# crabml/crabml

Hardware: AMD Instinct MI355X
Metric: decode tokens/sec (batch-1 greedy), Llama-3-8B shape Q4_0 (higher is better)
Workload: dtype q4_0 x q8_0 -> i32 dot, f32 accumulate

## Files before the change

crabml_amd/csrc/fused.hip:

```cpp
#include <algorithm>
#include <chrono>
#include <thread>
#include <cmath>

#include "fused_common.hpp"
#include "fused_attention.hpp"
#include "fused_ffn.hpp"
#include "sampler.hpp"
#include "prefill_rows.hpp"
#include "lazy.hpp"


#include <dlfcn.h>

using namespace crabml_hip;

struct crabml_hip_tp_comm {
  crabml_hip_device* dev = nullptr;
  void* nccl = nullptr;
  int nranks = 1, rank = 0;
  bool p2p = false;
  bool connected = false;
  unsigned long long* inbox = nullptr;
  bool via_ipc[8] = {false};
// ... 214 lines not shown
  return t;
}

hipError_t raise_dyn_lds(const crabml_hip_device* dev, const void* fn, int bytes) {
  static std::mutex mu;
  static std::map<std::pair<int, const void*>, int> have;
  if (dev->dry) return hipErrorNoDevice;
  std::lock_guard<std::mutex> g(mu);
  int& cur = have[{dev->ordinal, fn}];
  if (bytes <= cur) return hipSuccess;
  const hipError_t e = hipFuncSetAttribute(fn, hipFuncAttributeMaxDynamicSharedMemorySize, bytes);
  if (e == hipSuccess) cur = bytes;
  return e;
}

int dalloc(crabml_hip_llama* c, size_t bytes, void** out) {
  size_t cap = 0;
  CH_TRY(pool_alloc(c->dev, bytes, out, &cap));
  c->allocs.push_back({*out, cap});
  return 0;
}

Planes planes_of(const crabml_hip_buf* b) {
  return Planes{(const i32x4*)b->ptr, scale_plane<unsigned short>(b)};
}

struct ActPtrs {
  signed char* q;
  unsigned short* d;
  void* isum;
};
ActPtrs act_ptrs(char* p, size_t n, uint32_t qt) {
  ActLayout al = act_layout(qt, n);
  return ActPtrs{(signed char*)p, (unsigned short*)(p + al.off_d), (void*)(p + al.off_aux)};
}
template <int FMT>
typename ActOf<FMT>::type act_view(const ActPtrs& a) {
  ActLayout al;
  al.off_d = (size_t)((const char*)a.d - (const char*)a.q);
  al.off_aux = (size_t)((const char*)a.isum - (const char*)a.q);
  return act_at<typename ActOf<FMT>::type>((const char*)a.q, al);
}

int n_segments(const crabml_hip_llama* c) { return 2 * (int)c->cfg.n_layers + 1; }

int chunk_split(uint64_t flags, int k, int dim, int n_cu, bool x_only = false) {
  return (flags & CRABML_HIP_LLAMA_SPLIT_CHUNKS_ALWAYS)  ? 2
         : (flags & CRABML_HIP_LLAMA_SPLIT_CHUNKS_NEVER) ? 1
         : (k / 32 >= 256 && dim / 32 <= n_cu)           ? 2
         : (x_only && dim / 32 <= n_cu)                  ? 2
                                                         : 1;
}

int norm_nit(int dim) { return dim <= 4096 ? 4 : 12; }
void launch_norm_f32(hipStream_t st, float* x, const float* addv, const float* wn, int dim, float eps, float* out, int half) {
  with_const_else<4, 12>(norm_nit(dim), [&](auto nit) {
    k_norm_f32<decltype(nit)::value><<<1, 1024, norm_lds_bytes(dim), st>>>(x, addv, wn, dim, eps, out, half);
  });
}

typedef decltype(&k_attn_pv_split<1>) PvSplitFn;
struct PvSplitKernel {
  PvSplitFn fn = nullptr;
  int nsub = 0, threads = 0;
  size_t lds = 0;
};
PvSplitKernel pv_split_kernel(int grp) {
  PvSplitKernel k;
  with_const<1, 2, 4, 6, 8>(grp, [&](auto g) {
    typedef PvSplit<decltype(g)::value> P;
    k = PvSplitKernel{k_attn_pv_split<decltype(g)::value>, P::NSUB, P::THREADS, P::LDS};
  });
  return k;
}
typedef decltype(&k_attn_s<0>) AttnSFn;
AttnSFn attn_s_kernel(int hd) { return hd == 128 ? k_attn_s<128> : k_attn_s<0>; }
typedef decltype(&k_attn_flash_rows<64>) FlashRowsFn;
FlashRowsFn flash_rows_kernel(int hd) { return hd == 128 ? k_attn_flash_rows<128> : hd == 64 ? k_attn_flash_rows<64> : nullptr; }
typedef decltype(&k_gemv_res_nq<CRABML_HIP_Q4_K, 1, 1, false, false, true>) NqOrdKFn;
NqOrdKFn nq_ord_k_kernel(int split, int qin) {
  NqOrdKFn fn = nullptr;
  with_const_else<2, 1>(split, [&](auto s) {
    with_const_else<2, 1>(qin, [&](auto q) { fn = k_gemv_res_nq<CRABML_HIP_Q4_K, decltype(s)::value, decltype(q)::value, false, false, true>; });
  });
  return fn;
}
typedef FmtList<CRABML_HIP_Q4_K, CRABML_HIP_Q5_K, CRABML_HIP_Q6_K, CRABML_HIP_Q3_K, CRABML_HIP_Q2_K> KBodies;
struct KBodyRow {
  int fmt;
  bool epi_only;
  bool v_whole;
  int n_alt;
  int alt[2];
  bool takes(uint32_t t) const {
    for (int i = 0; i < n_alt; i++)
      if ((uint32_t)alt[i] == t) return true;
    return false;
  }
};
template <int FMT, int... ALT>
constexpr KBodyRow k_body_row(FmtList<ALT...>) {
  return KBodyRow{FMT, KBody<FMT>::EPI_ONLY, KBody<FMT>::V_WHOLE, (int)sizeof...(ALT), {ALT...}};
}
template <int... FMTS>
const KBodyRow* k_body_of(FmtList<FMTS...>, uint32_t t) {
  static constexpr KBodyRow rows[] = {k_body_row<FMTS>(typename KBody<FMTS>::VAlt{})...};
// ... 240 lines not shown
      k_sample_pick<true><<<1, SAMPLE_PICK_THREADS, 0, st>>>(c->sm_keys, n, c->sm_hist, ss);
    else
      k_sample_pick<false><<<1, SAMPLE_PICK_THREADS, 0, st>>>(c->sm_keys, n, c->sm_hist, ss);
    CH_HIP(dev, hipGetLastError());
    return 0;
  }
  k_argmax_partial<<<ARGMAX_BLOCKS, 256, 0, st>>>(out, c->vocab_l, c->am_val, c->am_idx, c->vocab_off);
  if (c->split_vocab && c->comm && c->comm->p2p)
    k_argmax_step_tp<<<1, 64, 0, st>>>(c->am_val, c->am_idx, ARGMAX_BLOCKS, token_d, pos_d, step_d, c->out_tokens, c->out_cap, c->state + 4,
                                       tp_view(c, true), n_segments(c));
  else
    k_argmax_step<<<1, 64, 0, st>>>(c->am_val, c->am_idx, ARGMAX_BLOCKS, token_d, pos_d, step_d, c->out_tokens, c->out_cap, c->state + 4,
                                    c->split_vocab ? c->am_best : (int*)nullptr);
  CH_HIP(dev, hipGetLastError());
  return 0;
}

static QkvEpiB qwen2_epi(const crabml_hip_llama* c, const QkvEpi& e, int l) {
  return QkvEpiB{e, (const float*)c->bq[l]->ptr, (const float*)c->bk[l]->ptr, (const float*)c->bv[l]->ptr};
}
template <class E>
struct QkvArchOf {
  static constexpr int value = QKV_LLAMA;
};
template <>
struct QkvArchOf<QkvEpiB> {
  static constexpr int value = QKV_QWEN2;
};
template <>
struct QkvArchOf<QkvEpiN> {
  static constexpr int value = QKV_GEMMA;
};
template <class F>
void with_qkv_epi(const crabml_hip_llama* c, const QkvEpi& e, int l, F&& f) {
  if (c->qwen2)
    f(qwen2_epi(c, e, l));
  else if (c->gemma)
    f(QkvEpiN{e});
  else
    f(e);
}
QkvEpi decode_qkv_epi(const crabml_hip_llama* c, int l) {
  return QkvEpi{c->qbuf, c->kc[l], c->vc[l], c->rope, c->state + 1, 1.0f / std::sqrt((float)c->hd), c->dim_l, c->kv_dim_l, c->hd,
                (int)c->cfg.rope_dim, c->npairs, (int)c->cfg.seq_len, c->cfg.use_f16_kv_cache ? 1 : 0};
}
void launch_embed(const crabml_hip_llama* c) {
  const int dim = (int)c->cfg.embedding_dim;
  k_embed<<<(dim + 255) / 256, 256, 0, c->dev->stream>>>((const char*)c->token_embed->ptr, (int)c->token_embed->dtype,
                                                         c->token_embed->wl.off_scale, c->state, dim, c->x, c->embed_scale);
}

template <int QIN, bool TP = false, bool DEFER = false>
struct NqForm {};
template <int FMT, int SPLIT, int QIN, bool TP, bool DEFER>
constexpr auto nq_kernel(NqForm<QIN, TP, DEFER>) {
  return &k_gemv_res_nq<FMT, SPLIT, QIN, TP, DEFER>;
}

template <int FMT>
int enqueue_segment_t(crabml_hip_llama* c, int seg) {
  crabml_hip_device* dev = c->dev;
  hipStream_t st = dev->stream;
  const auto& g = c->cfg;
  const int dim = (int)g.embedding_dim, hd = c->hd;
  const int dim_l = c->dim_l, kv_dim_l = c->kv_dim_l, hidden_l = c->hidden_l;
  const int n_heads_l = c->n_heads_l;
  const bool tp = c->tp > 1;
  const int L = (int)g.n_layers;
  constexpr bool Q81 = FMT == CRABML_HIP_Q4_1;
  const uint32_t qt = c->qt;
  ActPtrs ad = act_ptrs(c->act_dim, dim, qt), aa = act_ptrs(c->act_attn, dim_l, qt), ah = act_ptrs(c->act_hid, hidden_l, qt);
  const bool prof = dev->prof_on && !c->use_graph && !c->capturing;
  const double blk_b = (double)block_bytes(c->wtype) / 32.0;
  auto P0 = [&](crabml_hip_device::ProfRec* r, uint32_t stage, double rows, double k) {
    return prof ? prof_begin(dev, r, c->wtype, stage, rows * k * blk_b + 4.0 * k + 4.0 * rows) : 0;
  };
  auto P1 = [&](crabml_hip_device::ProfRec* r) { return prof ? prof_end(dev, r) : 0; };
  crabml_hip_device::ProfRec pr{};
  crabml_hip_device::ProfRec* R = prof ? &pr : nullptr;
  const bool do_pf = !(g.flags & CRABML_HIP_LLAMA_NO_PREFETCH);
  auto plan = [&](const crabml_hip_buf* a, const crabml_hip_buf* b, const crabml_hip_buf* cc) {
    PrefetchPlan pf{};
    const crabml_hip_buf* v[3] = {a, b, cc};
    for (int i = 0; i < 3; i++) {
      pf.p[i] = do_pf && v[i] ? v[i]->ptr : nullptr;
      pf.n[i] = do_pf && v[i] ? (v[i]->wl.total / 16) * 16 : 0;
    }
    pf.sink = c->state + 3;
    return pf;
  };
  const int spare = do_pf ? (dev->n_cu > 1 ? dev->n_cu - 1 : 0) : 0;
  const size_t norm_lds = norm_lds_bytes(dim);
  auto norm_quant = [&](const float* wn, float eps, bool add_pending, const PrefetchPlan& pf) {
    crabml_hip_device::ProfRec nr{};
    if (prof) prof_begin(dev, &nr, CRABML_HIP_F32, 6, 8.0 * dim);
    const float* addv = add_pending ? c->partial : nullptr;
    with_const_else<4, 12>(norm_nit(dim), [&](auto nit) {
      launch_k(st, prof ? &nr : nullptr, k_norm_quant<decltype(nit)::value, Q81>, dim3(1 + spare), dim3(1024), norm_lds, c->x, addv, wn, dim, eps, ad.q,
               ad.d, ad.isum, pf, c->plan.ordered ? 0 : 1);
    });
    if (prof) prof_end(dev, &nr);
  };
  const bool norm_epi = c->plan.norm_epi;
  static const int qkv_upfront = test_hook_off("CRABML_HIP_QKV_UPFRONT") ? 0 : 1;
  const bool defer_wo = c->plan.defer_norm && !Q81;
  const bool defer_down = c->plan.defer_norm && !Q81;
  auto gemv_out = [&](const crabml_hip_buf* w, const ActPtrs& a, int k, uint32_t stage, const float* wnext, float eps_next, bool defer = false,
                      const float* xin = nullptr) -> int {
    CH_TRY(P0(&pr, stage, dim, k));
    float* dst = tp ? c->partial : c->x;
    if (norm_epi) {
      NormGather ng{c->slots, c->slots + dim / 16, c->state + 4, c->state + 5, n_segments(c), seg, c->rsums};
      const int split = chunk_split(g.flags, k, dim, dev->n_cu);
      c->tap.note(seg / 2, stage == 2 ? CRABML_HIP_PLAN_SPLIT_WO : CRABML_HIP_PLAN_SPLIT_DOWN, split);
      const TpP2P tpv = tp_view(c, tp);
      auto nq = [&](auto form, size_t lds, const float* rhs, auto tparg) {
        with_const_else<2, 1>(split, [&](auto s) {
          launch_k(st, R, nq_kernel<FMT, decltype(s)::value>(form), dim3(dim / 32 * split), dim3(1024), lds, planes_of(w), act_view<FMT>(a), rhs, c->x,
                   wnext, eps_next, ad.q, ad.d, ad.isum, ng, k / 32, Planes6{nullptr, 0}, tparg);
        });
      };
      if (xin != nullptr && !Q81) {
        if constexpr (!Q81) {
          if (tpv.n > 1)
            nq(NqForm<1, true>{}, q8_0_lds_bytes(k / 32), xin, tpv);
          else
            nq(NqForm<1>{}, q8_0_lds_bytes(k / 32), xin, NoTp{});
        }
      } else if (tpv.n > 1) {
        nq(NqForm<0, true>{}, 0, nullptr, tpv);
      } else if (c->plan.ordered) {
        static const int pipe_mode = test_hook_int("CRABML_HIP_ORD_PIPE", -1);
        const int pipe = pipe_mode >= 0 ? pipe_mode : FMT == CRABML_HIP_Q8_0 ? 2 : 1;
        const bool piped = pipe >= (split == 2 ? 1 : 2);
        with_const_else<2, 1>(split, [&](auto s) {
          with_const_else<0, 1>(piped, [&](auto p) {
            launch_k(st, R, k_gemv_res_nq_ord<FMT, decltype(s)::value, decltype(p)::value != 0>, dim3(dim / 32 * split), dim3(1024),
                     nq_ord_lds_bytes(k / 32, split), planes_of(w), act_view<FMT>(a), c->x, wnext, eps_next, ad.q, ad.d, ad.isum, ng, k / 32);
          });
        });
      } else if (defer && !Q81) {
        if constexpr (!Q81) nq(NqForm<0, false, true>{}, 0, nullptr, NoTp{});
      } else {
        nq(NqForm<0>{}, 0, nullptr, NoTp{});
      }
    } else if (c->plan.ordered) {
      launch_k(st, R, k_gemv_res_ord<FMT>, dim3((dim + 7) / 8), dim3(256), ord_terms_lds_bytes(k / 32), planes_of(w), act_view<FMT>(a), c->x, dim, k / 32);
    } else if (tp) {
      launch_k(st, R, k_gemv_res<FMT, 1, false>, dim3((dim + 1) / 2), dim3(128), 0, planes_of(w), act_view<FMT>(a), dst, dim, k / 32);
    } else {
      launch_k(st, R, k_gemv_res<FMT, 1, true>, dim3((dim + 1) / 2), dim3(128), 0, planes_of(w), act_view<FMT>(a), dst, dim, k / 32);
    }
    CH_TRY(P1(&pr));
    return 0;
  };

  const size_t ad_bytes = act_layout(qt, (size_t)dim).total, rs_bytes = c->rsums ? (size_t)(dim / 32) * 4 : 0;
  TapRec& tap = c->tap;
  auto TAP = [&](bool on, int f, const void* src, size_t bytes) -> int { return on ? tap.copy(c, f, src, bytes) : 0; };
  if (seg == 2 * L) {
    const void* cls_act = c->act_dim;
    if (c->out_qt != qt) {
      const float* addv = tp && !norm_epi ? c->partial : nullptr;
      launch_norm_f32(st, c->x, addv, (const float*)c->rms_final->ptr, dim, g.rms_norm_eps, c->xn, c->plan.ordered ? 0 : 1);
      if (c->out_qt == CRABML_HIP_F32) {
        cls_act = c->xn;
      } else {
        launch_quantize_act(st, c->out_qt, c->xn, (size_t)dim, c->act_dim);
      }
    } else if (!norm_epi) {
      norm_quant((const float*)c->rms_final->ptr, g.rms_norm_eps, tp, plan(nullptr, nullptr, nullptr));
      CH_TRY(TAP(tap.layer == L - 1, CRABML_HIP_TAP_DOWN_ACT, c->act_dim, ad_bytes));
// ... 2278 lines not shown
```

crabml_amd/csrc/fused_ffn.hpp:

```cpp
#pragma once
#include "fused_common.hpp"

namespace crabml_hip {
template <int FMT, int R, bool ADD>
__global__ __launch_bounds__(128) void k_gemv_res(Planes w, typename ActOf<FMT>::type act, float* __restrict__ x, int m, int nb) {
  const int lane = threadIdx.x & 63;
  const int wave = blockIdx.x * (blockDim.x >> 6) + wave_in_wg();
  const int row0 = wave * R;
  if (row0 >= m) return;
  float res[R];
#pragma unroll
  for (int r = 0; r < R; r++) res[r] = (ADD && lane == 0 && row0 + r < m) ? x[row0 + r] : 0.f;
  float acc[R];
  rows_dot<FMT, R>(w.q, w.d, act, row0, m, nb, lane, acc);
#pragma unroll
  for (int r = 0; r < R; r++) {
    float s = wave_sum_f32(acc[r]);
    if (lane == 0 && row0 + r < m) x[row0 + r] = ADD ? s + res[r] : s;
  }
}

template <int FMT>
__global__ __launch_bounds__(256) void k_gemv_res_ord(Planes w, typename ActOf<FMT>::type act, float* __restrict__ x, int m, int nb) {
  extern __shared__ __attribute__((aligned(16))) float ord_terms[];
// ... 99 lines not shown
      if (sb >= nsb) break;
      const Q8KLane o = q8k_wave_quant(v[u], lane);
      if (cm)
        q8k_store_class_major((signed char*)sq + sb * 256, lane, o.packed);
      else
        sq[sb * 64 + lane] = o.packed;
      if ((lane & 3) == 0) sbs[sb * 16 + (lane >> 2)] = (short)o.quad_sum;
      if (lane == 0) sd[sb] = o.d;
    }
  }
  __syncthreads();
}

__device__ __forceinline__ void stage_copy_q8k(const ActQ8_K& act, int nsb, i32x4* sq, float* sd, short* sbs, bool cm) {
  const i32x4* src = cm ? act.qp : act.q;
  for (int i = threadIdx.x; i < nsb * 16; i += blockDim.x) sq[i] = src[i];
  for (int i = threadIdx.x; i < nsb; i += blockDim.x) sd[i] = act.d[i];
  for (int i = threadIdx.x; i < nsb * 2; i += blockDim.x) ((i32x4*)sbs)[i] = ((const i32x4*)act.bsums)[i];
  __syncthreads();
}

struct StageQ8Regs {
  float v[4];
};
__device__ __forceinline__ StageQ8Regs stage_quant_q8_0_request(const float* __restrict__ x, int nb, int b0) {
  const int lane = threadIdx.x & 63, nw = blockDim.x >> 6;
  const int l32 = lane & 31, hf = lane >> 5;
  StageQ8Regs r;
#pragma unroll
  for (int u = 0; u < 4; u++) {
    const int b = b0 + u * 2 * nw + hf;
    r.v[u] = x[(size_t)(b < nb ? b : nb - 1) * 32 + l32];
  }
  return r;
}
__device__ __forceinline__ void stage_quant_q8_0_store(const StageQ8Regs& r, int nb, int b0, signed char* sq, unsigned short* sd, int* ss) {
  const int lane = threadIdx.x & 63, nw = blockDim.x >> 6;
  const int l32 = lane & 31, hf = lane >> 5;
#pragma unroll
  for (int u = 0; u < 4; u++) {
    if (b0 + u * 2 * nw >= nb) break;
    const int b = b0 + u * 2 * nw + hf;
    const QLane o = quant_lane32<false>(r.v[u], true);
    if (b < nb) {
      sq[b * 32 + l32] = o.q;
      if (l32 == 0) {
        sd[b] = o.d;
        ss[b] = o.aux;
      }
    }
  }
}
__host__ __device__ inline size_t q8_0_lds_bytes(int nb) { return (size_t)nb * 32 + (size_t)((nb + 1) & ~1) * 2 + (size_t)nb * 4; }
__host__ __device__ inline size_t q8k_lds_bytes(int k) { return (size_t)k + (size_t)(k / 256) * 4 + (size_t)(k / 16) * 2; }
__host__ __device__ inline size_t q8k_ord_lds_bytes(int k, int rows) {
  return ((q8k_lds_bytes(k) + 15) & ~(size_t)15) + (size_t)rows * (size_t)q4k_rec_stride(k / 256) * sizeof(float);
}

struct NormGather {
  unsigned long long* slots;
  unsigned long long* pair;
  const int* serial;
  int* fault;
  int nseg, seg;
  float* sums;
  signed char* qp = nullptr;
};
__device__ __forceinline__ unsigned long long ld_granule(const unsigned long long* p) {
  return __hip_atomic_load(p, __ATOMIC_RELAXED, __HIP_MEMORY_SCOPE_AGENT);
}
template <int FMT, int SPLIT, bool TP = false, bool DEFER = false, bool ORD = false>
__device__ __forceinline__ void nq_epilogue(float (&acc)[2 / SPLIT], float res, float wn, f32x4 wn4, unsigned epoch, float* hv,
                                            float* __restrict__ x, signed char* __restrict__ q, void* __restrict__ d,
                                            void* __restrict__ isum, const NormGather& ng, float eps, int blk, int part, int nchunks,
                                            int row, int lane, int wave, int wg_index, int nwg_all,
                                            const typename TpArg<TP>::type& tp = typename TpArg<TP>::type{}) {
  constexpr bool Q81 = FMT == CRABML_HIP_Q4_1;
  constexpr bool KQ = FMT == CRABML_HIP_Q4_K;
  constexpr int RW = 2 / SPLIT;
  constexpr int ROWS = 32 / SPLIT;
  constexpr bool ROWG = SPLIT > 1 || KQ;
  static_assert(!ORD || (KQ && !TP && !DEFER), "the ordered epilogue: Q4_K layers on one device");
  if constexpr (!ORD) {
#pragma unroll
    for (int r = 0; r < RW; r++) {
      const float s = wave_sum_f32(acc[r]);
      if (lane == 0) hv[part * ROWS + wave * RW + r] = s;
    }
  }
  __syncthreads();
  if (wave != 0) return;
  if (lane < ROWS) {
    float mo = hv[part * ROWS + lane];
    if constexpr (TP) mo = tp_allreduce_elem(tp, mo, row + lane, epoch + tp.salt, ng.seg & 1);
    const float xv = mo + res;
    x[row + lane] = xv;
    hv[part * ROWS + lane] = xv;
    if (ROWG && q != nullptr)
      __hip_atomic_store(ng.pair + row + lane, ((unsigned long long)epoch << 32) | (unsigned long long)__builtin_bit_cast(unsigned, xv),
                         __ATOMIC_RELAXED, __HIP_MEMORY_SCOPE_AGENT);
  }
  __builtin_amdgcn_fence(__ATOMIC_RELEASE, "workgroup");
  __builtin_amdgcn_wave_barrier();
  auto poll = [&](const unsigned long long* p) -> float {
    unsigned long long g = ld_granule(p);
    int tries = 0;
// ... 116 lines not shown
    for (int i = 0; i < 4; i++) v4[i] = (unsigned)(g[i] >> 32) == epoch ? __builtin_bit_cast(float, (unsigned)g[i]) : poll(p + i);
  } else if (SPLIT > 1) {
    if (lane < 32) v = own ? hv[l32] : poll(ng.pair + blk * 32 + l32);
  } else {
    v = hv[l32];
  }
  float sum = 0.0f;
  const int nwg = nwg_all;
  for (int base = 0; base < nchunks; base += 64) {
    const int c = base + lane;
    float cv;
    if constexpr (ORD) {
      cv = c < nchunks ? poll(ng.slots + (SPLIT > 1 ? 2 * c + 1 : c)) : 0.0f;
#pragma unroll
      for (int i = 0; i < 64; i++) sum += rl_f(cv, i);
      continue;
    }
    if (SPLIT > 1) {
      const float h0 = c < nchunks ? poll(ng.slots + 2 * c) : 0.0f;
      const float h1 = c < nchunks ? poll(ng.slots + 2 * c + 1) : 0.0f;
      cv = h0 + h1;
    } else {
      cv = c < nchunks ? poll(ng.slots + c) : 0.0f;
    }
    sum += wave_sum_f32(cv);
  }
  (void)nwg;
  const float rms = sqrtf(sum / (float)(nchunks * 32) + eps);
  if constexpr (!KQ) {
    const float xn = (v / rms) * wn;
    const QLane o = quant_lane32<Q81>(xn, true);
    if (lane < 32 && own) {
      q[blk * 32 + lane] = o.q;
      if (lane == 0) {
        ((unsigned short*)d)[blk] = o.d;
        store_qaux<Q81>(isum, blk, o.aux);
      }
    }
  } else {
    f32x4 xn;
#pragma unroll
    for (int i = 0; i < 4; i++) xn[i] = (v4[i] / rms) * wn4[i];
    const Q8KLane o = q8k_wave_quant(xn, lane);
    const int l0 = (blk & 7) * 8 + part * (ROWS / 4);
    if (lane >= l0 && lane < l0 + ROWS / 4) {
      ((unsigned*)q)[sb * 64 + lane] = o.packed;
      q8k_store_class_major(ng.qp + sb * 256, lane, o.packed);
      if ((lane & 3) == 0) ((short*)isum)[sb * 16 + (lane >> 2)] = (short)o.quad_sum;
    }
    if (lane == 0 && (blk & 7) == 0 && part == 0) ((float*)d)[sb] = o.d;
  }
}

template <int FMT, int SPLIT, int QIN = 0, bool TP = false, bool DEFER = false, bool ORD = false>
__global__ __launch_bounds__(1024) void k_gemv_res_nq(Planes w, typename ActOf<FMT>::type act, const float* __restrict__ xin,
                                                      float* __restrict__ x,
                                                      const float* __restrict__ wnext, float eps,
                                                      signed char* __restrict__ q, void* __restrict__ d,
                                                      void* __restrict__ isum, NormGather ng, int nb, Planes6 w6,
                                                      typename TpArg<TP>::type tp) {
  constexpr bool KQ = KBody<FMT>::IS;
  constexpr int EF = KQ ? CRABML_HIP_Q4_K : FMT;
  constexpr bool W6 = kbody_takes_q6k<FMT>;
  static_assert(!KBody<FMT>::EPI_ONLY || (!TP && !DEFER && !ORD), "a K-quant body of the norm-epilogue form only: the fast step on one device");
  constexpr int RW = 2 / SPLIT;
  constexpr int ROWS = 32 / SPLIT;
  __shared__ __attribute__((aligned(16))) float hv[32];
  const int lane = threadIdx.x & 63, wave = wave_in_wg();
  const int blk = blockIdx.x / SPLIT, part = blockIdx.x % SPLIT;
  const int nchunks = gridDim.x / SPLIT;
  const int row = blk * 32 + part * ROWS + wave * RW;
  float res = 0.f;
  float wn = 0.f;
  f32x4 wn4 = {0.f, 0.f, 0.f, 0.f};
  unsigned epoch = 0;
  if (wave == 0) {
    if (lane < ROWS) res = x[row + lane];
    if constexpr (KQ)
      wn4 = ((const f32x4*)wnext)[(blk >> 3) * 64 + lane];
    else
      wn = wnext[blk * 32 + (lane & 31)];
  }
  if (wave == 0) epoch = (unsigned)(*ng.serial) * (unsigned)ng.nseg + (unsigned)ng.seg + 1u;
  float acc[RW];
  if constexpr (KQ && QIN) {
    extern __shared__ i32x4 lds_act[];
    float* sd = (float*)(lds_act + nb * 16);
    short* sbs = (short*)(sd + nb);
    if (W6 && w6.base != nullptr) {
      if constexpr (QIN == 2)
        stage_copy_q8k(act, nb, lds_act, sd, sbs, false);
      else
        stage_quant_q8k(xin, nb, (unsigned*)lds_act, sd, sbs, false);
      const ActQ8_K la6{lds_act, sd, sbs, lds_act};
      if constexpr (ORD) {
        const int stride = q4k_rec_stride(nb);
        float* T = (float*)((char*)lds_act + (((size_t)nb * 292 + 15) & ~(size_t)15));
        rows_terms_q6k<RW>(w6.base, w6.off_qh, la6, row, nchunks * 32, nb, lane, T + (size_t)(wave * RW) * stride, stride);
        __syncthreads();
        if (wave == 0 && lane < ROWS) hv[part * ROWS + lane] = q4k_ordered_sum(T + (size_t)lane * stride, nb);
        nq_epilogue<EF, SPLIT, TP, false, true>(acc, res, wn, wn4, epoch, hv, x, q, d, isum, ng, eps, blk, part, nchunks, row, lane, wave,
                                                (int)blockIdx.x, (int)gridDim.x, tp);
        return;
      }
      rows_partial_q6k<RW>(w6.base, w6.off_qh, la6, row, nchunks * 32, nb, lane, acc);
      nq_epilogue<EF, SPLIT, TP>(acc, res, wn, wn4, epoch, hv, x, q, d, isum, ng, eps, blk, part, nchunks, row, lane, wave,
                                 (int)blockIdx.x, (int)gridDim.x, tp);
// ... 63 lines not shown
  } else if constexpr (QIN == 1) {
    static_assert(KQ || QIN != 1 || FMT == CRABML_HIP_Q4_0 || FMT == CRABML_HIP_Q8_0, "Q8_0 rhs");
    using F = BlockFmt<FMT>;
    extern __shared__ i32x4 lds_act[];
    signed char* sq = (signed char*)lds_act;
    unsigned short* sd = (unsigned short*)(sq + (size_t)nb * 32);
    int* ss = (int*)(sd + ((nb + 1) & ~1));
#pragma unroll
    for (int r = 0; r < RW; r++) acc[r] = 0.f;
    const int nu = nb * F::UNITS;
    typename F::Blk ka0[RW], kb0[RW];
    const int ua = lane < nu ? lane : nu - 1, ub = lane + 64 < nu ? lane + 64 : nu - 1;
    const int nw16 = (int)(blockDim.x >> 6);
    StageQ8Regs hq = stage_quant_q8_0_request(xin, nb, wave * 2);
#pragma unroll
    for (int r = 0; r < RW; r++) {
      ka0[r] = F::load(w.q, w.d, (size_t)(row + r), nb, ua);
      kb0[r] = F::load(w.q, w.d, (size_t)(row + r), nb, ub);
    }
    for (int b0 = wave * 2; b0 < nb; b0 += 8 * nw16) {
      if (b0 != wave * 2) hq = stage_quant_q8_0_request(xin, nb, b0);
      stage_quant_q8_0_store(hq, nb, b0, sq, sd, ss);
    }
    __syncthreads();
    const ActQ8_0 la{(const i32x4*)sq, sd, ss};
    if (lane < nu) {
      const XUnit xa = F::loadx(la, ua);
#pragma unroll
      for (int r = 0; r < RW; r++) acc[r] += F::term(ka0[r], xa);
    }
    if (lane + 64 < nu) {
      const XUnit xb = F::loadx(la, ub);
#pragma unroll
      for (int r = 0; r < RW; r++) acc[r] += F::term(kb0[r], xb);
    }
    for (int u = lane + 128; u < nu; u += 128) {
      const int u2 = u + 64;
      const bool two = u2 < nu;
      const int uu = two ? u2 : u;
      typename F::Blk ka[RW], kb[RW];
#pragma unroll
      for (int r = 0; r < RW; r++) {
        ka[r] = F::load(w.q, w.d, (size_t)(row + r), nb, u);
        kb[r] = F::load(w.q, w.d, (size_t)(row + r), nb, uu);
      }
      const XUnit xa = F::loadx(la, u), xb = F::loadx(la, uu);
#pragma unroll
      for (int r = 0; r < RW; r++) acc[r] += F::term(ka[r], xa);
      if (two) {
#pragma unroll
        for (int r = 0; r < RW; r++) acc[r] += F::term(kb[r], xb);
      }
    }
  } else {
    using F = BlockFmt<FMT>;
#pragma unroll
    for (int r = 0; r < RW; r++) acc[r] = 0.f;
    const int nu = nb * F::UNITS;
    for (int u = lane; u < nu; u += 128) {
      const int u2 = u + 64;
      const bool two = u2 < nu;
      const int uu = two ? u2 : u;
      typename F::Blk ka[RW], kb[RW];
#pragma unroll
      for (int r = 0; r < RW; r++) {
        ka[r] = F::load(w.q, w.d, (size_t)(row + r), nb, u);
        kb[r] = F::load(w.q, w.d, (size_t)(row + r), nb, uu);
      }
      const XUnit xa = F::loadx(act, u), xb = F::loadx(act, uu);
#pragma unroll
      for (int r = 0; r < RW; r++) acc[r] += F::term(ka[r], xa);
      if (two) {
#pragma unroll
        for (int r = 0; r < RW; r++) acc[r] += F::term(kb[r], xb);
      }
    }
  }
  nq_epilogue<EF, SPLIT, TP, DEFER>(acc, res, wn, wn4, epoch, hv, x, q, d, isum, ng, eps, blk, part, nchunks, row, lane, wave,
                                    (int)blockIdx.x, (int)gridDim.x, tp);
}

__host__ __device__ inline size_t nq_ord_lds_bytes(int nb, int split) { return (size_t)(32 / split) * (((nb + 3) & ~3) + 4) * sizeof(float); }
template <int FMT, int SPLIT, bool PIPE>
__global__ __launch_bounds__(1024) void k_gemv_res_nq_ord(Planes w, typename ActOf<FMT>::type act, float* __restrict__ x,
                                                          const float* __restrict__ wnext, float eps, signed char* __restrict__ q,
                                                          void* __restrict__ d, void* __restrict__ isum, NormGather ng, int nb) {
  constexpr bool Q81 = FMT == CRABML_HIP_Q4_1;
  constexpr int RW = 2 / SPLIT, ROWS = 32 / SPLIT;
  extern __shared__ __attribute__((aligned(16))) float ord_terms[];
  __shared__ __attribute__((aligned(16))) float hv[32];
  const int lane = threadIdx.x & 63, wave = wave_in_wg();
  const int blk = blockIdx.x / SPLIT, part = blockIdx.x % SPLIT;
  const int nchunks = gridDim.x / SPLIT;
  const int row_wg = blk * 32 + part * ROWS;
  float res = 0.f, wn = 0.f;
  unsigned epoch = 0;
  if (wave == 0) {
    if (lane < ROWS) res = x[row_wg + lane];
    wn = wnext[blk * 32 + (lane & 31)];
    epoch = (unsigned)(*ng.serial) * (unsigned)ng.nseg + (unsigned)ng.seg + 1u;
  }
  const int nt = ((nb + 3) & ~3) + 4;
  __shared__ int prog[16];
  if (PIPE) {
    if (lane == 0) prog[wave] = 0;
    __syncthreads();
// ... 561 lines not shown
```

crabml_amd/csrc/gemv_core.hpp:

```cpp
#pragma once
#include <type_traits>

#include "devutil.hpp"

namespace crabml_hip {

__device__ __forceinline__ int dot_q4_0(i32x4 q, i32x4 xlo, i32x4 xhi, int xsum) {
  int s = 0;
#pragma unroll
  for (int i = 0; i < 4; i++) {
    int w = q[i];
    s = __builtin_amdgcn_sdot4(w & 0x0F0F0F0F, xlo[i], s, false);
    s = __builtin_amdgcn_sdot4((w >> 4) & 0x0F0F0F0F, xhi[i], s, false);
  }
  return s - 8 * xsum;
}
__device__ __forceinline__ int dot_u4(i32x4 q, i32x4 xlo, i32x4 xhi) {
  int s = 0;
#pragma unroll
  for (int i = 0; i < 4; i++) {
    int w = q[i];
    s = __builtin_amdgcn_sdot4(w & 0x0F0F0F0F, xlo[i], s, false);
    s = __builtin_amdgcn_sdot4((w >> 4) & 0x0F0F0F0F, xhi[i], s, false);
  }
// ... 130 lines not shown
  static __device__ __forceinline__ XUnit loadx(const ActQ8_1& act, int u) {
    return XUnit{act.q[2 * u], act.q[2 * u + 1], 0.0f, (int)((unsigned)act.d[u] | ((unsigned)act.s[u] << 16))};
  }
  static __device__ __forceinline__ float term(const Blk& b, const XUnit& x) {
    const int si = dot_u4(b.q, x.x0, x.x1);
    const unsigned short dwh = (unsigned short)(b.dm & 0xffffu), mwh = (unsigned short)(b.dm >> 16);
    const unsigned short dxh = (unsigned short)((unsigned)x.xs & 0xffffu), sxh = (unsigned short)((unsigned)x.xs >> 16);
    return h2f(h_mul(dwh, dxh)) * (float)si + h2f(h_mul(mwh, sxh));
  }
};

template <int FMT, int R, class ACT>
__device__ __forceinline__ void rows_partial(const i32x4* __restrict__ wq, const unsigned short* __restrict__ wd,
                                             const ACT& act, int row0, int m, int nb, int lane, float acc[R], int rs = 1) {
  using F = BlockFmt<FMT>;
#pragma unroll
  for (int r = 0; r < R; r++) acc[r] = 0.f;
  const int nu = nb * F::UNITS;
  for (int u = lane; u < nu; u += 64) {
    typename F::Blk blk[R];
#pragma unroll
    for (int r = 0; r < R; r++) {
      int row = row0 + r * rs < m ? row0 + r * rs : m - 1;
      blk[r] = F::load(wq, wd, (size_t)row, nb, u);
    }
    const XUnit x = F::loadx(act, u);
#pragma unroll
    for (int r = 0; r < R; r++) acc[r] += F::term(blk[r], x);
  }
}

template <int FMT, int R, class ACT>
__device__ __forceinline__ void rows_partial_2step(const i32x4* __restrict__ wq, const unsigned short* __restrict__ wd, const ACT& act,
                                                   int row0, int m, int nb, int lane, float acc[R], int rs = 1) {
  using F = BlockFmt<FMT>;
#pragma unroll
  for (int r = 0; r < R; r++) acc[r] = 0.f;
  const int nu = nb * F::UNITS;
  for (int u = lane; u < nu; u += 128) {
    typename F::Blk b0[R], b1[R];
#pragma unroll
    for (int r = 0; r < R; r++) {
      const int row = row0 + r * rs < m ? row0 + r * rs : m - 1;
      b0[r] = F::load(wq, wd, (size_t)row, nb, u);
      b1[r] = F::load(wq, wd, (size_t)row, nb, u + 64);
    }
    const XUnit x0 = F::loadx(act, u), x1 = F::loadx(act, u + 64);
#pragma unroll
    for (int r = 0; r < R; r++) {
      acc[r] += F::term(b0[r], x0);
      acc[r] += F::term(b1[r], x1);
    }
  }
}

template <int FMT, int R, class ACT>
__device__ __forceinline__ float rows_partial_rms(const i32x4* __restrict__ wq, const unsigned short* __restrict__ wd, const ACT& act,
                                                  int row0, int m, int nb, int lane, float acc[R], const RmsTail& rt, RmsReq rq,
                                                  int rs = 1) {
  using F = BlockFmt<FMT>;
#pragma unroll
  for (int r = 0; r < R; r++) acc[r] = 0.f;
  const int nu = nb * F::UNITS;
  float inv_rms = 1.0f;
  for (int u0 = 0; u0 < nu; u0 += 64) {
    const int u = u0 + lane;
    const bool live = u < nu;
    const int uu = live ? u : nu - 1;
    typename F::Blk blk[R];
#pragma unroll
    for (int r = 0; r < R; r++) {
      int row = row0 + r * rs < m ? row0 + r * rs : m - 1;
      blk[r] = F::load(wq, wd, (size_t)row, nb, uu);
    }
    const XUnit x = F::loadx(act, uu);
    if (u0 == 0) {
      __builtin_amdgcn_sched_barrier(0);
      asm volatile("" : "+v"(rq.v0), "+v"(rq.v1));
      inv_rms = rms_finish(rt, rq, lane);
    }
#pragma unroll
    for (int r = 0; r < R; r++) {
      const float t = F::term(blk[r], x);
      acc[r] += live ? t : 0.0f;
    }
  }
  return inv_rms;
}

template <int FMT, int R, class ACT>
__device__ __forceinline__ float rows_partial_rms_128(const i32x4* __restrict__ wq, const unsigned short* __restrict__ wd, const ACT& act,
                                                      int row0, int m, int nb, int lane, float acc[R], const RmsTail& rt, RmsReq rq,
                                                      int rs = 1) {
  using F = BlockFmt<FMT>;
  typename F::Blk b0[R], b1[R];
#pragma unroll
  for (int r = 0; r < R; r++) {
    const int row = row0 + r * rs < m ? row0 + r * rs : m - 1;
    b0[r] = F::load(wq, wd, (size_t)row, nb, lane);
    b1[r] = F::load(wq, wd, (size_t)row, nb, lane + 64);
  }
  const XUnit x0 = F::loadx(act, lane), x1 = F::loadx(act, lane + 64);
  __builtin_amdgcn_sched_barrier(0);
  asm volatile("" : "+v"(rq.v0), "+v"(rq.v1));
  const float inv_rms = rms_finish(rt, rq, lane);
#pragma unroll
// ... 1026 lines not shown
```

include/crabml_hip_debug.h:

```cpp
#ifndef CRABML_HIP_DEBUG_H
#define CRABML_HIP_DEBUG_H

#include "crabml_hip.h"

#ifdef __cplusplus
extern "C" {
#endif

#define CRABML_HIP_FLAG_LAZY_NO_FUSION 4
#define CRABML_HIP_FLAG_DRY 0x40000000
int crabml_hip_debug_lazy_stats(crabml_hip_device_t* dev, uint64_t* out, size_t cap);

int crabml_hip_debug_device_numa_node(crabml_hip_device_t* dev, int32_t* node);

int crabml_hip_debug_quantize(crabml_hip_device_t* dev, const crabml_hip_buf_t* x, size_t n, uint32_t qtype,
                              void* dst, size_t dst_bytes);
int crabml_hip_debug_block_dots(crabml_hip_device_t* dev, const crabml_hip_buf_t* w, size_t m, size_t k, size_t row,
                                const crabml_hip_buf_t* x, int32_t* dst);
int crabml_hip_debug_superblock_ints(crabml_hip_device_t* dev, const crabml_hip_buf_t* w, size_t m, size_t k, size_t row,
                                     const crabml_hip_buf_t* x, int32_t variant, int32_t* dst, float* value);
int crabml_hip_debug_gemm_ints(crabml_hip_device_t* dev, const crabml_hip_buf_t* w, size_t m, size_t k,
                               const crabml_hip_buf_t* x, size_t b, int32_t* dst, float* out);
int crabml_hip_debug_gemm_f16w(crabml_hip_device_t* dev, const crabml_hip_buf_t* const* w, const size_t* m, size_t nw, size_t k,
                               const crabml_hip_buf_t* x, size_t b, int32_t rows_path, uint16_t junk, const int32_t* force,
                               float* const* out, uint16_t* xh, int32_t* used, void* hq, uint16_t* hxh);
int crabml_hip_debug_read_ceiling(crabml_hip_device_t* dev, size_t bytes, int32_t reps, double* gbytes_per_s);

int crabml_hip_debug_flash_attention(crabml_hip_device_t* dev, const float* q, const uint16_t* k, const uint16_t* v, size_t n_heads,
                                     size_t n_kv, size_t head_dim, size_t seq, size_t slices, float* out, float* out2);

int crabml_hip_debug_flash_attention_rows(crabml_hip_device_t* dev, const float* q, const uint16_t* k, const uint16_t* v, size_t n_heads,
                                          size_t n_kv, size_t head_dim, size_t pos0, size_t rows, size_t seq_cap, float* out);

int crabml_hip_debug_sample(crabml_hip_device_t* dev, const float* logits, size_t n, float temperature, float topp, float coin,
                            uint32_t* token);

#define CRABML_HIP_LLAMA_NO_NORM_EPILOGUE 4
#define CRABML_HIP_LLAMA_NO_KQUANT_FUSION 256
#define CRABML_HIP_LLAMA_Q4_1_SEGMENTS 512
#define CRABML_HIP_LLAMA_NO_TILE_ATTENTION 2048
#define CRABML_HIP_LLAMA_NO_RHS_PROLOGUE 1024
#define CRABML_HIP_LLAMA_TP_DRY_RUN 128
#define CRABML_HIP_LLAMA_NO_LONG_ATTENTION 64
#define CRABML_HIP_LLAMA_NO_Q8K_PRODUCERS 32768
#define CRABML_HIP_LLAMA_Q8K_ATTN_PRODUCER 65536
#define CRABML_HIP_LLAMA_NO_PV_PRODUCER_WAVES 131072
#define CRABML_HIP_LLAMA_NO_PREFILL_ROW_FUSION 262144
#define CRABML_HIP_LLAMA_NO_PV_ROW_TILES 16384
#define CRABML_HIP_LLAMA_NO_STAGED_ATTENTION 8192
#define CRABML_HIP_LLAMA_FLASH_TICKET 2097152
#define CRABML_HIP_LLAMA_NO_H_CONSUMER_QUANT 4096
#define CRABML_HIP_LLAMA_PREFILL_INT8_GEMM 524288
#define CRABML_HIP_LLAMA_PREFILL_SEPARATE_F16_ROWS 33554432
#define CRABML_HIP_LLAMA_PREFILL_NO_GU_EPILOGUE 67108864
#define CRABML_HIP_LLAMA_NO_K_NORM_IN 16777216
#define CRABML_HIP_LLAMA_SPLIT_CHUNKS_ALWAYS 16
#define CRABML_HIP_LLAMA_SPLIT_CHUNKS_NEVER 32

int crabml_hip_llama_debug_kv(crabml_hip_llama_t* ctx, size_t layer, int32_t which_v, void* dst, size_t nbytes);

enum {
  CRABML_HIP_TAP_QKV_IN_X = 0,
  CRABML_HIP_TAP_QKV_IN_ACT = 1,
  CRABML_HIP_TAP_QKV_IN_RSUMS = 2,
  CRABML_HIP_TAP_QBUF = 3,
  CRABML_HIP_TAP_ATTN = 4,
  CRABML_HIP_TAP_ACT_ATTN = 5,
  CRABML_HIP_TAP_WO_X = 6,
  CRABML_HIP_TAP_WO_ACT = 7,
  CRABML_HIP_TAP_WO_RSUMS = 8,
  CRABML_HIP_TAP_ACT_HID = 9,
  CRABML_HIP_TAP_DOWN_X = 10,
  CRABML_HIP_TAP_DOWN_ACT = 11,
  CRABML_HIP_TAP_DOWN_RSUMS = 12,
  CRABML_HIP_TAP_CLS_ACT = 13,
  CRABML_HIP_TAP_PLAN = 14,
  CRABML_HIP_TAP_GATEUP_H = 15,
  CRABML_HIP_TAP_QKV_IN_XN = 16,
  CRABML_HIP_TAP_WO_XN = 17,
  CRABML_HIP_TAP_CLS_XN = 18,
  CRABML_HIP_TAP_QKV_IN_QP = 19,
  CRABML_HIP_TAP_ACT_ATTN_QP = 20,
  CRABML_HIP_TAP_WO_QP = 21,
  CRABML_HIP_TAP_ACT_HID_QP = 22,
  CRABML_HIP_TAP_DOWN_QP = 23,
  CRABML_HIP_TAP_CLS_QP = 24,
  CRABML_HIP_TAP_FIELDS = 25
};
enum {
  CRABML_HIP_PLAN_N_CU = 0,
  CRABML_HIP_PLAN_DEFER_NORM = 1,
  CRABML_HIP_PLAN_NORM_EPILOGUE = 2,
  CRABML_HIP_PLAN_ATTN_VARIANT = 3,
  CRABML_HIP_PLAN_SPLIT_WO = 4,
  CRABML_HIP_PLAN_SPLIT_DOWN = 5,
  CRABML_HIP_PLAN_QKV_LOADER = 6,
  CRABML_HIP_PLAN_NORM_NIT = 7,
  CRABML_HIP_PLAN_PATH = 8,
  CRABML_HIP_PLAN_NORM_EPI_K = 9,
  CRABML_HIP_PLAN_Q8K_PRODUCERS = 10,
  CRABML_HIP_PLAN_K_NORM_IN = 11,
  CRABML_HIP_PLAN_QIN = 12,
  CRABML_HIP_PLAN_QMODE_WO = 13,
  CRABML_HIP_PLAN_QMODE_DOWN = 14,
  CRABML_HIP_PLAN_WO_X_ONLY = 15,
  CRABML_HIP_PLAN_AQ8 = 16,
  CRABML_HIP_PLAN_V_Q6K = 17,
  CRABML_HIP_PLAN_DOWN_Q6K = 18,
  CRABML_HIP_TAP_PLAN_WORDS = 19
};
// ... 132 lines not shown
```

Before: 680.2.

## Issue weight loads before staging activations in LDS for split residual GEMV

Adds a deep-prefetch variant of the residual norm-quant GEMV that loads the first two rounds of weight blocks into registers before it stages the Q8 activation vector into shared memory. Later rounds then keep a two-deep software pipeline of weight loads while reading activations from LDS. The goal is to hide global-load latency on the split-2 Wo/down projections and to stop every wave re-fetching activations from global memory. In exchange it uses more registers per wave and needs LDS plus a block-wide barrier. It applies only to the non-TP, non-prequantized-input, split-2 path and can be disabled with a new flag.

```diff
diff --git a/crabml_amd/csrc/fused.hip b/crabml_amd/csrc/fused.hip
--- a/crabml_amd/csrc/fused.hip
+++ b/crabml_amd/csrc/fused.hip
@@ -290,6 +290,11 @@
                                                          : 1;
 }
 
+int nq_request_depth(uint64_t flags, int k, int rows_per_wave, int waves_per_cu) {
+  if ((flags & CRABML_HIP_LLAMA_NQ_TWO_UNIT_ROUNDS) || rows_per_wave != 1 || waves_per_cu > 16 || k > ACT_STAGE_MAX_K) return 0;
+  return NQ_DEEP;
+}
+
 int norm_nit(int dim) { return dim <= 4096 ? 4 : 12; }
 void launch_norm_f32(hipStream_t st, float* x, const float* addv, const float* wn, int dim, float eps, float* out, int half) {
   with_const_else<4, 12>(norm_nit(dim), [&](auto nit) {
@@ -636,9 +641,9 @@
 
 template <int QIN, bool TP = false, bool DEFER = false>
 struct NqForm {};
-template <int FMT, int SPLIT, int QIN, bool TP, bool DEFER>
+template <int FMT, int SPLIT, int DEEP, int QIN, bool TP, bool DEFER>
 constexpr auto nq_kernel(NqForm<QIN, TP, DEFER>) {
-  return &k_gemv_res_nq<FMT, SPLIT, QIN, TP, DEFER>;
+  return &k_gemv_res_nq<FMT, SPLIT, QIN, TP, DEFER, false, QIN == 0 && SPLIT == 2 ? DEEP : 0>;
 }
 
 template <int FMT>
@@ -698,10 +703,15 @@
       const int split = chunk_split(g.flags, k, dim, dev->n_cu);
       c->tap.note(seg / 2, stage == 2 ? CRABML_HIP_PLAN_SPLIT_WO : CRABML_HIP_PLAN_SPLIT_DOWN, split);
       const TpP2P tpv = tp_view(c, tp);
+      const int nwg = dim / 32 * split;
+      const int depth = nq_request_depth(g.flags, k, 2 / split, (nwg + dev->n_cu - 1) / dev->n_cu * 16);
       auto nq = [&](auto form, size_t lds, const float* rhs, auto tparg) {
         with_const_else<2, 1>(split, [&](auto s) {
-          launch_k(st, R, nq_kernel<FMT, decltype(s)::value>(form), dim3(dim / 32 * split), dim3(1024), lds, planes_of(w), act_view<FMT>(a), rhs, c->x,
-                   wnext, eps_next, ad.q, ad.d, ad.isum, ng, k / 32, Planes6{nullptr, 0}, tparg);
+          with_const_else<NQ_DEEP, 0>(depth, [&](auto dp) {
+            launch_k(st, R, nq_kernel<FMT, decltype(s)::value, decltype(dp)::value>(form), dim3(nwg), dim3(1024),
+                     decltype(dp)::value > 0 && lds == 0 ? q8_0_lds_bytes(k / 32) : lds, planes_of(w), act_view<FMT>(a),
+                     rhs, c->x, wnext, eps_next, ad.q, ad.d, ad.isum, ng, k / 32, Planes6{nullptr, 0}, tparg);
+          });
         });
       };
       if (xin != nullptr && !Q81) {
diff --git a/crabml_amd/csrc/fused_ffn.hpp b/crabml_amd/csrc/fused_ffn.hpp
--- a/crabml_amd/csrc/fused_ffn.hpp
+++ b/crabml_amd/csrc/fused_ffn.hpp
@@ -175,6 +175,7 @@
   }
 }
 __host__ __device__ inline size_t q8_0_lds_bytes(int nb) { return (size_t)nb * 32 + (size_t)((nb + 1) & ~1) * 2 + (size_t)nb * 4; }
+constexpr int NQ_DEEP = 2;
 __host__ __device__ inline size_t q8k_lds_bytes(int k) { return (size_t)k + (size_t)(k / 256) * 4 + (size_t)(k / 16) * 2; }
 __host__ __device__ inline size_t q8k_ord_lds_bytes(int k, int rows) {
   return ((q8k_lds_bytes(k) + 15) & ~(size_t)15) + (size_t)rows * (size_t)q4k_rec_stride(k / 256) * sizeof(float);
@@ -397,7 +398,7 @@
   }
 }
 
-template <int FMT, int SPLIT, int QIN = 0, bool TP = false, bool DEFER = false, bool ORD = false>
+template <int FMT, int SPLIT, int QIN = 0, bool TP = false, bool DEFER = false, bool ORD = false, int DEEP = 0>
 __global__ __launch_bounds__(1024) void k_gemv_res_nq(Planes w, typename ActOf<FMT>::type act, const float* __restrict__ xin,
                                                       float* __restrict__ x,
                                                       const float* __restrict__ wnext, float eps,
@@ -567,6 +568,13 @@
         for (int r = 0; r < RW; r++) acc[r] += F::term(kb[r], xb);
       }
     }
+  } else if constexpr (DEEP > 0) {
+    extern __shared__ i32x4 lds_act[];
+    const ActStage stg = act_stage_request(act, nb);
+    rows_partial_deep<FMT, RW, DEEP>(w.q, w.d, act_stage_view(act, nb, lds_act), row, nchunks * 32, nb, lane, acc, [&]() {
+      act_stage_store(act, stg, nb, lds_act);
+      __syncthreads();
+    });
   } else {
     using F = BlockFmt<FMT>;
 #pragma unroll
diff --git a/crabml_amd/csrc/gemv_core.hpp b/crabml_amd/csrc/gemv_core.hpp
--- a/crabml_amd/csrc/gemv_core.hpp
+++ b/crabml_amd/csrc/gemv_core.hpp
@@ -206,6 +206,105 @@
       acc[r] += F::term(b1[r], x1);
     }
   }
+}
+
+
+__device__ __forceinline__ void pin_scale(unsigned short& d) {
+  unsigned s = d;
+  asm volatile("" : "+v"(s));
+  d = (unsigned short)s;
+}
+__device__ __forceinline__ void pin_scale(unsigned& dm) { asm volatile("" : "+v"(dm)); }
+
+template <int FMT, int R, int D, class ACT, class MID>
+__device__ __forceinline__ void rows_partial_deep(const i32x4* __restrict__ wq, const unsigned short* __restrict__ wd, const ACT& act,
+                                                  int row0, int m, int nb, int lane, float acc[R], MID mid) {
+  using F = BlockFmt<FMT>;
+#pragma unroll
+  for (int r = 0; r < R; r++) acc[r] = 0.f;
+  const int nu = nb * F::UNITS;
+  const int nsteps = (nu + 63) >> 6;
+  size_t rows[R];
+#pragma unroll
+  for (int r = 0; r < R; r++) rows[r] = (size_t)(row0 + r < m ? row0 + r : m - 1);
+  typename F::Blk blk[D][R];
+#pragma unroll
+  for (int j = 0; j < D; j++) {
+    const int u = j * 64 + lane, uu = u < nu ? u : nu - 1;
+#pragma unroll
+    for (int r = 0; r < R; r++) blk[j][r] = F::load(wq, wd, rows[r], nb, uu);
+  }
+  mid();
+  int s0 = 0;
+  for (; s0 + D < nsteps; s0 += D) {
+#pragma unroll
+    for (int j = 0; j < D; j++) {
+      const XUnit x = F::loadx(act, (s0 + j) * 64 + lane);
+#pragma unroll
+      for (int r = 0; r < R; r++) acc[r] += F::term(blk[j][r], x);
+      const int u = (s0 + D + j) * 64 + lane, uu = u < nu ? u : nu - 1;
+#pragma unroll
+      for (int r = 0; r < R; r++) blk[j][r] = F::load(wq, wd, rows[r], nb, uu);
+    }
+  }
+#pragma unroll
+  for (int j = 0; j < D; j++) {
+    if (s0 + j < nsteps) {
+      const int u = (s0 + j) * 64 + lane;
+      const bool live = u < nu;
+      const XUnit x = F::loadx(act, live ? u : nu - 1);
+#pragma unroll
+      for (int r = 0; r < R; r++) {
+        if constexpr (FMT == CRABML_HIP_Q4_1)
+          pin_scale(blk[j][r].dm);
+        else
+          pin_scale(blk[j][r].d);
+        const float t = F::term(blk[j][r], x);
+        acc[r] += live ? t : 0.0f;
+      }
+    }
+  }
+}
+
+constexpr int ACT_STAGE_MAX_K = 32768;
+struct ActStage {
+  i32x4 q0, q1;
+  unsigned short d;
+  int aux;
+};
+__device__ __forceinline__ int act_aux(const ActQ8_0& a, int b) { return a.isum[b]; }
+__device__ __forceinline__ int act_aux(const ActQ8_1& a, int b) { return (int)a.s[b]; }
+template <class ACT>
+__device__ __forceinline__ ActStage act_stage_request(const ACT& act, int nb) {
+  const int t = (int)threadIdx.x, nq = 2 * nb;
+  ActStage s{act.q[t < nq ? t : nq - 1], i32x4{0, 0, 0, 0}, act.d[t < nb ? t : nb - 1], act_aux(act, t < nb ? t : nb - 1)};
+  if (nq > 1024) s.q1 = act.q[t + 1024 < nq ? t + 1024 : nq - 1];
+  __builtin_amdgcn_sched_barrier(0);
+  return s;
+}
+__device__ __forceinline__ void act_stage_put(const ActStage& s, int nb, i32x4* sq, unsigned short* sd) {
+  const int t = (int)threadIdx.x, nq = 2 * nb;
+  if (t < nq) sq[t] = s.q0;
+  if (t + 1024 < nq) sq[t + 1024] = s.q1;
+  if (t < nb) sd[t] = s.d;
+}
+__device__ __forceinline__ ActQ8_0 act_stage_view(const ActQ8_0&, int nb, i32x4* lds) {
+  unsigned short* sd = (unsigned short*)(lds + 2 * nb);
+  return ActQ8_0{lds, sd, (const int*)(sd + ((nb + 1) & ~1))};
+}
+__device__ __forceinline__ ActQ8_1 act_stage_view(const ActQ8_1&, int nb, i32x4* lds) {
+  unsigned short* sd = (unsigned short*)(lds + 2 * nb);
+  return ActQ8_1{lds, sd, sd + ((nb + 1) & ~1)};
+}
+__device__ __forceinline__ void act_stage_store(const ActQ8_0&, const ActStage& s, int nb, i32x4* lds) {
+  unsigned short* sd = (unsigned short*)(lds + 2 * nb);
+  act_stage_put(s, nb, lds, sd);
+  if ((int)threadIdx.x < nb) ((int*)(sd + ((nb + 1) & ~1)))[threadIdx.x] = s.aux;
+}
+__device__ __forceinline__ void act_stage_store(const ActQ8_1&, const ActStage& s, int nb, i32x4* lds) {
+  unsigned short* sd = (unsigned short*)(lds + 2 * nb);
+  act_stage_put(s, nb, lds, sd);
+  if ((int)threadIdx.x < nb) (sd + ((nb + 1) & ~1))[threadIdx.x] = (unsigned short)s.aux;
 }
 
 template <int FMT, int R, class ACT>
diff --git a/include/crabml_hip_debug.h b/include/crabml_hip_debug.h
--- a/include/crabml_hip_debug.h
+++ b/include/crabml_hip_debug.h
@@ -56,6 +56,7 @@
 #define CRABML_HIP_LLAMA_NO_K_NORM_IN 16777216
 #define CRABML_HIP_LLAMA_SPLIT_CHUNKS_ALWAYS 16
 #define CRABML_HIP_LLAMA_SPLIT_CHUNKS_NEVER 32
+#define CRABML_HIP_LLAMA_NQ_TWO_UNIT_ROUNDS 134217728
 
 int crabml_hip_llama_debug_kv(crabml_hip_llama_t* ctx, size_t layer, int32_t which_v, void* dst, size_t nbytes);
 
```

Result: faster. 688.7 (median of 6 runs) (+1.3%).
